# eridgd/WCT-TF

Measured on AMD Instinct MI355X. Metric: stylized frames/sec @512x512, 5-level relu5->1 pipeline, alpha=0.8, higher is better.
Workload: dtype f16

## Files before the change

### wct_tf_amd/csrc/api.hip

```cpp
#include "common.h"
#include "../../include/wct_hip.h"

#include <stdarg.h>
#include <stdio.h>
#include <string.h>
#include <stdlib.h>
#include <vector>
#include <cmath>
#include <algorithm>

static thread_local char g_err[512] = "";
void wct_set_error(const char* fmt, ...) {
  va_list ap;
  va_start(ap, fmt);
  vsnprintf(g_err, sizeof(g_err), fmt, ap);
  va_end(ap);
}
extern "C" const char* wct_last_error(void) { return g_err; }

struct DevBuf {
  void* p = nullptr;
  size_t cap = 0;
};

// ... 458 lines not shown
  ProfScope ps(c, conv3x3_wino_takes(a) ? 9 : 0, 2.0 * px * 9 * l.cin * l.cout,
               in_px * l.cin * 2 + out_px * l.cout * ((y16 ? 2 : 0) + (y32 ? 4 : 0)) + 9.0 * l.cin * l.cout * 2);
  return launch_conv3x3(a, c->stream);
}

static int run_encoder(wct_ctx* c, const float* img, int B, int H, int W, int clamp01, int deepest,
                       float* const taps32[6], float* const* usum = nullptr, unsigned* const* umax = nullptr) {
  if (!c->enc_loaded) { wct_set_error("encoder weights not set (wct_set_encoder)"); return WCT_ERR_STATE; }
  ARG_CHECK(deepest >= 1 && deepest <= 5 && H >= 2 && W >= 2);
  const size_t act_bytes = (size_t)B * H * W * 64 * sizeof(half_t);
  TRY(ensure(c, c->act[0], act_bytes));
  TRY(ensure(c, c->act[1], act_bytes));
  half_t* cur = (half_t*)c->act[0].p;
  half_t* nxt = (half_t*)c->act[1].p;
  static const int fuse_conv1_env = getenv("WCT_FUSE_CONV1") ? atoi(getenv("WCT_FUSE_CONV1")) : 1;
  const bool fuse_conv1 = fuse_conv1_env && deepest > 1 && !taps32[1];
  if (!fuse_conv1) {
    ConvFirstArgs a;
    a.x = img; a.wfrag = c->first_w; a.bias = c->first_b;
    a.y16 = deepest > 1 ? cur : nullptr; a.y32 = taps32[1];
    a.B = B; a.H = H; a.W = W; a.clamp01 = clamp01;
    a.usum = usum && taps32[1] ? usum[1] : nullptr; a.umax = a.usum ? umax[1] : nullptr;
    const double px = (double)B * H * W;
    ProfScope ps(c, 1, 2.0 * px * 27 * 64, px * (12 + 64 * ((a.y16 ? 2 : 0) + (a.y32 ? 4 : 0))));
    TRY(launch_conv_first(a, c->stream));
  }
  if (deepest == 1) return WCT_OK;
  static const int seq_tap[12] = {0, 2, 0, 3, 0, 0, 0, 4, 0, 0, 0, 5};
  static const int pool_after[12] = {1, 0, 1, 0, 0, 0, 1, 0, 0, 0, 1, 0};
  int h = H, w = W;
  for (int i = 0; i < 12; ++i) {
    const ConvLayer& l = c->enc[i];
    const int tap = seq_tap[i];
    const bool last = tap == deepest;
    const bool fuse = pool_after[i];
    float* const us = tap && taps32[tap] && usum ? usum[tap] : nullptr;
    if (i == 0 && fuse_conv1) {
      ConvArgs a;
      a.x = nullptr; a.w = l.w; a.bias = l.b; a.y16 = nxt; a.y32 = nullptr; a.usum = nullptr; a.umax = nullptr;
// ... 54 lines not shown
  const int mode = (flags & WCT_FLAG_MODE_NP) ? WCT_MODE_NP : WCT_MODE_TF;
  {
    ProfScope ps(c, 4, cost.cov_flops, cost.cov_bytes);
    TRY(launch(mode, WCT_STAGE_COV));
  }
  {
    ProfScope ps(c, 5, 0, 0);
    TRY(launch(mode, WCT_STAGE_EIG));
  }
  ProfScope ps(c, 6, cost.apply_flops, cost.apply_bytes);
  return launch(mode, WCT_STAGE_APPLY);
}

static int run_transform(wct_ctx* c, const float* fc, int Nc, const float* fs, int Ns, int C, int P,
                         float alpha, unsigned flags, float eps, half_t* out16, float* out32, int* sweeps_dev,
                         const WctFeatStats* st = nullptr) {
  const int shared = (flags & WCT_FLAG_STYLE_SHARED) ? 1 : 0;
  const StageCost cost = {(double)P * 2.0 * C * C * ((double)Nc + Ns), (double)P * 2.0 * ((double)Nc + Ns) * C * 4,
                          (double)P * (2.0 * C * C * Nc + 6.0 * C * C * C), (double)P * Nc * C * (4 + (out16 ? 2 : 0) + (out32 ? 4 : 0)),
                          (double)P * (2.0 * Nc + 2.0 * Ns) * C * 4 + (double)P * Nc * C * 6};
  return run_stages(c, wct_workspace_bytes(C, Nc, Ns, P), flags, cost, [&](int mode, int stages) {
    if (!stages) return launch_adain(fc, Nc, fs, Ns, C, P, alpha, 1e-5f, out16, out32, c->wct_ws.p, c->wct_ws.cap, c->stream, shared, st);
    return launch_wct(fc, Nc, fs, Ns, C, P, alpha, mode, eps, out16, out32, c->wct_ws.p, c->wct_ws.cap, sweeps_dev, stages, c->stream,
                      shared, c->eig_fail_dev, st);
  });
}

static int mix_weights(const float* weights, int K, float* lambda) {
  if (K < 1 || K > WCT_MIX_MAX) { wct_set_error("style mix: K = %d styles, must be 1 .. %d", K, (int)WCT_MIX_MAX); return WCT_ERR_ARG; }
  if (!weights) { wct_set_error("style mix: no weights"); return WCT_ERR_ARG; }
  double sum = 0.0;
  for (int k = 0; k < K; ++k) {
    if (!(weights[k] >= 0.f) || !std::isfinite(weights[k])) {
      wct_set_error("style mix: weight %d is %g; weights must be finite and >= 0", k, (double)weights[k]);
      return WCT_ERR_ARG;
    }
    sum += weights[k];
  }
  if (!(sum > 0.0) || !std::isfinite(sum)) { wct_set_error("style mix: the weights sum to %g, must be > 0", sum); return WCT_ERR_ARG; }
// ... 460 lines not shown
  if (flags & WCT_FLAG_IMAGES_F32) return WCT_OK;
  TRY(ensure(c, c->img_c, nc * 4));
  TRY(ensure(c, c->img_s, ns * 4));
  ProfScope ps(c, 7, 0, (double)(nc + ns) * 5);
  TRY(launch_u8_to_f32((const uint8_t*)content, (float*)c->img_c.p, nc, c->stream));
  TRY(launch_u8_to_f32((const uint8_t*)style, (float*)c->img_s.p, ns, c->stream));
  *img_c = (const float*)c->img_c.p; *img_s = (const float*)c->img_s.p;
  return WCT_OK;
}

static bool fuse_stats() {
  static const int on = getenv("WCT_FUSE_STATS") ? atoi(getenv("WCT_FUSE_STATS")) : 1;
  return on != 0;
}

template <typename StyleAt, typename Transform>
static int stylize_levels(wct_ctx* c, const float* img_c, int B, int Hc, int Wc, const int* levels, int n_levels, unsigned flags,
                          size_t umax_clear, int clear_from, StyleAt&& style_at, Transform&& transform, uint8_t* out) {
  unsigned* const umax_c = (unsigned*)c->umax.p;
  const float* cur = img_c;
  int H = Hc, W = Wc;
  for (int i = 0; i < n_levels; ++i) {
    const int l = levels[i], C = LEVEL_C[l];
    int h, w;
    level_dims(H, W, l, &h, &w);
    TRY(ensure(c, c->feat_c, (size_t)B * h * w * C * 4));
    float* ctaps[6] = {nullptr, nullptr, nullptr, nullptr, nullptr, nullptr};
    ctaps[l] = (float*)c->feat_c.p;
    float* us_c[6] = {nullptr, nullptr, nullptr, nullptr, nullptr, nullptr};
    unsigned* um_c[6] = {nullptr, nullptr, nullptr, nullptr, nullptr, nullptr};
    if (fuse_stats() && w % 16 == 0) {
      TRY(ensure(c, c->usum_c, (size_t)B * h * (w / 16) * C * 4));
      us_c[l] = (float*)c->usum_c.p; um_c[l] = umax_c;
      if (i >= clear_from) HIP_TRY(hipMemsetAsync(umax_c, 0, umax_clear, c->stream));
    }
    WctFeatStats st = {};
    st.u[0] = us_c[l]; st.umax[0] = um_c[l];
    TRY(run_encoder(c, cur, B, H, W, i > 0, l, ctaps, us_c, um_c));
    TRY(ensure(c, c->wct_out, (size_t)B * h * w * C * 2));
    if (l == 5 && (flags & WCT_FLAG_SWAP5)) {
      int hs, ws;
      style_at(l, 0, &hs, &ws);
      ARG_CHECK(h >= c->ss_patch && w >= c->ss_patch && hs >= c->ss_patch && ws >= c->ss_patch);
// ... 24 lines not shown
  int deepest, Ho, Wo;
  TRY(stylize_checks(c, Hc, Wc, &style, &Hs, &Ws, 1, levels, n_levels, &deepest, &Ho, &Wo));

  const int shared = (flags & WCT_FLAG_STYLE_SHARED) ? 1 : 0;
  const int Bs = shared ? 1 : B;
  const float *img_c, *img_s;
  TRY(images_f32(c, flags, content, (size_t)B * Hc * Wc * 3, style, (size_t)Bs * Hs * Ws * 3, &img_c, &img_s));
  const bool want_stats = fuse_stats();
  constexpr size_t UROW = 32 * UMAX_SLOTS;
  TRY(ensure(c, c->umax, 7 * UROW * sizeof(unsigned)));
  unsigned* const umax_c = (unsigned*)c->umax.p;
  if (want_stats) HIP_TRY(hipMemsetAsync(c->umax.p, 0, 7 * UROW * sizeof(unsigned), c->stream));
  float* taps[6] = {nullptr, nullptr, nullptr, nullptr, nullptr, nullptr};
  float* us_s[6] = {nullptr, nullptr, nullptr, nullptr, nullptr, nullptr};
  unsigned* um_s[6] = {nullptr, nullptr, nullptr, nullptr, nullptr, nullptr};
  for (int i = 0; i < n_levels; ++i) {
    const int l = levels[i];
    int h, w;
    level_dims(Hs, Ws, l, &h, &w);
    TRY(ensure(c, c->feat_s[l], (size_t)Bs * h * w * LEVEL_C[l] * 4));
    taps[l] = (float*)c->feat_s[l].p;
    if (want_stats && w % 16 == 0) {
      TRY(ensure(c, c->usum_s[l], (size_t)Bs * h * (w / 16) * LEVEL_C[l] * 4));
      us_s[l] = (float*)c->usum_s[l].p; um_s[l] = umax_c + UROW * l;
    }
  }
  TRY(run_encoder(c, img_s, Bs, Hs, Ws, 0, deepest, taps, us_s, um_s));

  auto style_at = [&](int l, int b, int* hs, int* ws) {
    level_dims(Hs, Ws, l, hs, ws);
    return (const float*)c->feat_s[l].p + (size_t)(shared ? 0 : b) * *hs * *ws * LEVEL_C[l];
  };
  return stylize_levels(c, img_c, B, Hc, Wc, levels, n_levels, flags, UROW * sizeof(unsigned), 1, style_at,
                        [&](int, int l, int C, int h, int w, WctFeatStats st) {
                          int hs, ws;
                          const float* fs = style_at(l, 0, &hs, &ws);
                          st.u[1] = us_s[l]; st.umax[1] = um_s[l];
                          return run_transform(c, (float*)c->feat_c.p, h * w, fs, hs * ws, C, B, alpha, flags, -1.f,
                                               (half_t*)c->wct_out.p, nullptr, nullptr, &st);
                        }, out);
}

extern "C" int wct_stylize(wct_ctx* c, const uint8_t* content, int Hc, int Wc, const uint8_t* style, int Hs, int Ws,
                           const int* levels, int n_levels, float alpha, unsigned flags, uint8_t* out) {
  ARG_CHECK(c && content && style && out);
  HIP_TRY(hipSetDevice(c->device));
  TRY(eig_stale(c));
  int Ho, Wo;
  TRY(wct_output_size(Hc, Wc, levels, n_levels, &Ho, &Wo));
  void *dc, *ds;
  const size_t px = (flags & WCT_FLAG_IMAGES_F32) ? sizeof(float) : 1;
  TRY(stage_in(c, 0, content, (size_t)Hc * Wc * 3 * px, &dc));
  TRY(stage_in(c, 1, style, (size_t)Hs * Ws * 3 * px, &ds));
  TRY(ensure(c, c->stage[2], (size_t)Ho * Wo * 3));
  TRY(wct_stylize_batch_dev(c, (uint8_t*)dc, Hc, Wc, (uint8_t*)ds, Hs, Ws, 1, levels, n_levels, alpha, flags,
// ... 383 lines not shown
```

### wct_tf_amd/csrc/common.h

```cpp
#pragma once
#include <hip/hip_runtime.h>
#include <stdint.h>
#include <stddef.h>

typedef _Float16 half_t;
typedef _Float16 half8 __attribute__((ext_vector_type(8)));
typedef _Float16 half4 __attribute__((ext_vector_type(4)));
typedef float f32x16 __attribute__((ext_vector_type(16)));
typedef float f32x4 __attribute__((ext_vector_type(4)));

#define WCT_OK 0
#define WCT_ERR_HIP -1
#define WCT_ERR_ARG -2
#define WCT_ERR_STATE -3
#define WCT_ERR_NOMEM -4
#define WCT_ERR_NOCONV -5

void wct_set_error(const char* fmt, ...);

#define HIP_TRY(expr)                                                          \
  do {                                                                         \
    hipError_t _e = (expr);                                                    \
    if (_e != hipSuccess) {                                                    \
      wct_set_error("%s failed: %s (%s:%d)", #expr, hipGetErrorString(_e),     \
// ... 106 lines not shown
  int nsplit;
  size_t sA, sB, s_sub_m, s_sub_n, s_sub_k, s_scale_k, s_out, s_bias;
  const float* A_odd;
  size_t sA_odd;
  int skip_shared;
  int blend; float alpha; unsigned* mabs;
  const float* mask_diag; size_t s_mask; int* mask_out; const int* mask_in;
};

int launch_gemm(GemmArgs g, int nsplit, int nbatch, hipStream_t s);

enum { WCT_MODE_NP = 0, WCT_MODE_TF = 1 };

struct WctFeatStats { const float* u[2]; const unsigned* umax[2]; };

size_t wct_workspace_bytes(int C, int Nc, int Ns, int P);
int launch_wct(const float* content, int Nc, const float* style, int Ns, int C, int P,
               float alpha, int mode, float eps , half_t* out16, float* out32,
               void* workspace, size_t workspace_bytes, int* sweeps_dev, int stages, hipStream_t s,
               int shared_style ,
               int* eig_fail ,
               const struct WctFeatStats* stats = nullptr );
enum { WCT_STAGE_COV = 1, WCT_STAGE_EIG = 2, WCT_STAGE_APPLY = 4, WCT_STAGE_ALL = 7, WCT_STAGE_EIG_FP32UPDATE = 8 };
int launch_adain(const float* content, int Nc, const float* style, int Ns, int C, int P,
                 float alpha, float eps, half_t* out16, float* out32,
                 void* workspace, size_t workspace_bytes, hipStream_t s, int shared_style,
                 const struct WctFeatStats* stats = nullptr);
enum { WCT_MIX_MAX = 8 };
size_t wct_mix_workspace_bytes(int C, int Nc, const int* Ns, int K, const float* lambda);
int launch_wct_mix(const float* content, int Nc, const float* const* styles, const int* Ns, int K, const float* lambda, int C,
                   float alpha, int mode, float eps, half_t* out16, float* out32, void* workspace, size_t workspace_bytes,
                   int* sweeps_dev, int stages, hipStream_t s, int* eig_fail, const struct WctFeatStats* stats = nullptr);
int launch_adain_mix(const float* content, int Nc, const float* const* styles, const int* Ns, int K, const float* lambda, int C,
                     float alpha, float eps, half_t* out16, float* out32, void* workspace, size_t workspace_bytes, hipStream_t s,
                     const struct WctFeatStats* stats = nullptr);
struct MaskGeom { const uint8_t* mask; int Hm, Wm, w, stride; };
size_t mask_compact_workspace_bytes(int N);
// ... 50 lines not shown
```

### wct_tf_amd/csrc/conv.hip

```cpp
#include "common.h"

typedef unsigned int u32x4 __attribute__((ext_vector_type(4)));
constexpr int TW = 16;
constexpr int PITCH = 20;
constexpr int BK = 32;

__device__ __forceinline__ int reflect_idx(int i, int n) {
  if (i < 0) i = -i;
  if (i >= n) i = 2 * n - 2 - i;
  i = i < 0 ? 0 : i;
  return i >= n ? n - 1 : i;
}

template <int MT, int NT, bool POOL, bool OUT32>
__device__ __forceinline__ void conv_epilogue_t(const ConvArgs& p, f32x16 (&acc)[NT][MT], int b, int y0, int x0, int n0,
                                                int wm, int wn, int lane, const unsigned char* bias_lds) {
  typedef _Float16 h2 __attribute__((ext_vector_type(2)));
  constexpr int OOB = (int)0x80000000u;
  const int frag_px = lane & 15;
  const int frag_py = (lane & 31) >> 4;
  const int kgrp = lane >> 5;
  const int Ho = POOL ? (p.H + 1) / 2 : p.H, Wo = POOL ? (p.W + 1) / 2 : p.W;
  const unsigned img_elems = (unsigned)Ho * Wo * p.Cout;
  const __amdgpu_buffer_rsrc_t r16 = __builtin_amdgcn_make_buffer_rsrc(
// ... 581 lines not shown
    }
    __builtin_amdgcn_fence(__ATOMIC_RELEASE, "wavefront");
    __builtin_amdgcn_wave_barrier();
  }
  if (next) {
    __syncthreads();
    park();
    __syncthreads();
  }
  }
  if (p.usum) umax_merge(p.umax + b * UMAX_SLOTS, (int)blockIdx.x * 4 + wave, vmax, lane);
}

int launch_conv_first(const ConvFirstArgs& a, hipStream_t s) {
  ARG_CHECK(a.H > 1 && a.W > 1 && a.B > 0);
  ARG_CHECK(!a.usum || (a.y32 && a.umax && a.W % 16 == 0));
  const int strips_x = cdiv(a.W, 64), tiles_y = cdiv(a.H, 16);
  hipLaunchKernelGGL(conv_first_kernel, dim3(strips_x * tiles_y, a.B), dim3(256), 0, s, a, strips_x);
  HIP_TRY(hipGetLastError());
  return WCT_OK;
}

__global__ __launch_bounds__(256) void conv_last_kernel(ConvLastArgs p, int tiles_x) {
  constexpr int PP = 33;
  __shared__ float part[18 * 18 * PP];
  const int tid = threadIdx.x, lane = tid & 63, wave = tid >> 6;
  const int tx = blockIdx.x % tiles_x, ty = blockIdx.x / tiles_x;
  const int b = blockIdx.y;
  const int y0 = ty * 16, x0 = tx * 16;
  const half_t* xb = p.x + (size_t)b * p.H * p.W * 64;
  half8 wf[4];
// ... 130 lines not shown
```

### wct_tf_amd/csrc/stats_gemm.hip

```cpp
#include "wct_stages.h"


struct StatArgs {
  const float* x[2];
  int n[2];
  const float* u[2];
  const unsigned* umax[2];
  const float* mean;
  float* partial;
  float* absmax;
  int C, nslab;
  int shared_style;
};

__global__ __launch_bounds__(256) void colsum_kernel(StatArgs p) {
  __shared__ f32x4 red[256];
  const int mat = blockIdx.y, slab = blockIdx.x;
  if (skip_style_mat(mat, p.shared_style)) return;
  const int b = mat & 1, pair = mat >> 1;
  const int C = p.C, cq = C / 4;
  const int nrp = 256 / cq;
  const int tid = threadIdx.x;
  const int rp = tid / cq, c4 = tid % cq;
  const int N = p.n[b];
// ... 489 lines not shown
    CovArgs ca;
    ca.x[0] = content; ca.x[1] = style; ca.n[0] = Nc; ca.n[1] = Ns;
    ca.mean = w.mean; ca.scale = w.scale; ca.partial = w.cov_partial;
    ca.C = C; ca.ksplit = w.ksplit; ca.nsplit = w.nsplit; ca.ntile = cdiv(C, BT); ca.shared_style = shared_style;
    dim3 grid(ca.ntile * (ca.ntile + 1) / 2, w.nsplit, 2 * P);
    if (BT == 128) hipLaunchKernelGGL((cov_f16x2_kernel<128>), grid, dim3(256), 0, s, ca);
    else hipLaunchKernelGGL((cov_f16x2_kernel<64>), grid, dim3(256), 0, s, ca);
    HIP_TRY(hipGetLastError());
  }
  hipLaunchKernelGGL(cov_finish_kernel, dim3(cdiv(C, 64), cdiv(C, 64), 2 * P), dim3(256), 0, s, w.cov_partial, w.scale, w.A, C,
                     w.nsplit, BT, 1.f / (float)(Nc - 1), 1.f / (float)(Ns - 1), eps, shared_style, w.A0);
  HIP_TRY(hipGetLastError());
  return WCT_OK;
}

static int launch_slot_means(const float* x, int N, int C, int m, int nslab, const WctCarve& w, bool with_var, hipStream_t s,
                             const float* u = nullptr, const unsigned* umax = nullptr) {
  StatArgs sa = {};
  sa.x[0] = sa.x[1] = x; sa.n[0] = sa.n[1] = N;
  sa.u[0] = umax ? u : nullptr; sa.umax[0] = sa.u[0] ? umax : nullptr;
  float* partial = w.stat_partial + (size_t)m * w.nslab * C;
  float* absmax = w.absmax + (size_t)m * w.nslab;
  sa.mean = nullptr; sa.partial = partial; sa.absmax = absmax; sa.C = C; sa.nslab = nslab; sa.shared_style = 0;
  hipLaunchKernelGGL(colsum_kernel, dim3(nslab, 1), dim3(256), 0, s, sa);
  hipLaunchKernelGGL(colsum_finish_kernel, dim3(cdiv(C, 256), 1), dim3(256), 0, s, partial, w.mean + (size_t)m * C, C, nslab, (float)N,
                     (float)N, 0, (const float*)absmax, w.scale + m);
  if (with_var) {
    sa.mean = w.mean + (size_t)m * C; sa.absmax = nullptr;
    hipLaunchKernelGGL(colsum_kernel, dim3(nslab, 1), dim3(256), 0, s, sa);
    hipLaunchKernelGGL(colsum_finish_kernel, dim3(cdiv(C, 256), 1), dim3(256), 0, s, partial, w.var + (size_t)m * C, C, nslab, (float)N,
// ... 33 lines not shown
```

### wct_tf_amd/csrc/wct.hip

```cpp
#include "wct_stages.h"
#include "jacobi_dev.h"
#include <algorithm>
#include <type_traits>



template <int BC, int BP, typename Args = ApplyArgs>
__global__ __launch_bounds__(256, 2) void apply_f16x2_kernel(Args p) {
  constexpr bool SEG = std::is_same<Args, ApplySegArgs>::value;
  constexpr int TM = BC / 64, TN = BP / 64;
  constexpr int MI = BC * 4 / 256, XI = BP * 4 / 256;
  __shared__ __attribute__((aligned(16))) unsigned char lm[2][BC * 64];
  __shared__ __attribute__((aligned(16))) unsigned char lx[2][BP * 64];
  typedef unsigned int u32x4 __attribute__((ext_vector_type(4)));
  const int tid = threadIdx.x, lane = tid & 63, wave = tid >> 6;
  const int wm = wave >> 1, wn = wave & 1;
  const int pair = blockIdx.z;
  const int n0 = blockIdx.x * BP, c0 = blockIdx.y * BC;
  int seg0 = 0, N = p.N;
  if constexpr (SEG) {
    seg0 = p.seg_off[p.lab[pair]];
    N = p.seg_off[p.lab[pair] + 1] - seg0;
    if (n0 >= N) return;
  }
// ... 134 lines not shown
        typedef _Float16 h2 __attribute__((ext_vector_type(2)));
        h2 lo = {(half_t)v[0], (half_t)v[1]}, hi = {(half_t)v[2], (half_t)v[3]};
        pk[rq][0] = __builtin_bit_cast(unsigned, lo);
        pk[rq][1] = __builtin_bit_cast(unsigned, hi);
      }
      if (p.out16) {
#pragma unroll
        for (int m = 0; m < 2; ++m) {
          auto sxw = __builtin_amdgcn_permlane32_swap(pk[2 * m][0], pk[2 * m + 1][0], false, false);
          auto syw = __builtin_amdgcn_permlane32_swap(pk[2 * m][1], pk[2 * m + 1][1], false, false);
          u32x4 o = {sxw[0], syw[0], sxw[1], syw[1]};
          const int co = cb + 16 * m + 8 * kgrp;
          if (n_ok && co < C) *reinterpret_cast<u32x4*>(p.out16 + row + co) = o;
        }
      }
    }
  }
}

int launch_apply_seg(const ApplySegArgs& a, int nmax, int P, hipStream_t s) {
  const int C = a.C;
  if (C >= 128) hipLaunchKernelGGL((apply_f16x2_kernel<128, 128, ApplySegArgs>), dim3(cdiv(nmax, 128), cdiv(C, 128), P), dim3(256), 0, s, a);
  else hipLaunchKernelGGL((apply_f16x2_kernel<64, 128, ApplySegArgs>), dim3(cdiv(nmax, 128), cdiv(C, 64), P), dim3(256), 0, s, a);
  HIP_TRY(hipGetLastError());
  return WCT_OK;
}

static int wct_nslab(int N) { int s = cdiv(N, 64); return s < 1 ? 1 : (s > 256 ? 256 : s); }

static void cov_split(int C, int Nmax, int P, int* nsplit, int* ksplit) {
// ... 52 lines not shown
size_t wct_workspace_bytes(int C, int Nc, int Ns, int P) {
  const int Cw = C < 32 ? 32 : C;
  return carve(nullptr, Cw, P, pair_layout(Cw, Nc, Ns)).total;
}

int launch_blend(const WctCarve& w, int C, int P, float alpha, int shared_style, hipStream_t s) {
  const size_t cc = (size_t)C * C;
  GemmArgs g = {};
  g.A = w.Tcs; g.lda = C; g.a_kmajor = 0; g.B = w.Tw; g.ldb = C; g.b_kmajor = 1; g.sA = shared_style ? 0 : 2 * cc; g.sB = 2 * cc;
  g.M = C; g.N = C; g.K = C; g.ksplit = C; g.out32 = w.M; g.ldo = C; g.s_out = cc;
  g.blend = 1; g.alpha = alpha; g.mabs = w.mabs;
  return launch_gemm(g, 1, P, s);
}

static int launch_blend_apply(const WctCarve& w, const float* content, int Nc, int C, int P, float alpha, int shared_style,
                              half_t* out16, float* out32, hipStream_t s) {
  int rc;
  if ((rc = launch_blend(w, C, P, alpha, shared_style, s))) return rc;
  {
    ApplyArgs a;
    a.x = content; a.N = Nc; a.C = C; a.mean = w.mean; a.M = w.M; a.bias = w.bias;
    a.xscale = w.scale; a.mabs = w.mabs; a.out16 = out16; a.out32 = out32;
    if (C >= 128) hipLaunchKernelGGL((apply_f16x2_kernel<128, 128>), dim3(cdiv(Nc, 128), cdiv(C, 128), P), dim3(256), 0, s, a);
    else hipLaunchKernelGGL((apply_f16x2_kernel<64, 128>), dim3(cdiv(Nc, 128), cdiv(C, 64), P), dim3(256), 0, s, a);
  }
  HIP_TRY(hipGetLastError());
  return WCT_OK;
}

int launch_wct(const float* content, int Nc, const float* style, int Ns, int C, int P, float alpha, int mode, float eps_in,
               half_t* out16, float* out32, void* workspace, size_t workspace_bytes, int* sweeps_dev,
               int stages, hipStream_t s, int shared_style, int* eig_fail, const WctFeatStats* stats) {
  ARG_CHECK(C % 32 == 0 && C >= 32 && C <= 1024 && Nc >= 2 && Ns >= 2 && P >= 1 && P <= 32);
  ARG_CHECK(mode == WCT_MODE_NP || mode == WCT_MODE_TF);
  ARG_CHECK((size_t)Nc * C * 4 < ((size_t)1 << 31) && (size_t)Ns * C * 4 < ((size_t)1 << 31));
  WctCarve w = carve(workspace, C, P, pair_layout(C, Nc, Ns));
  ARG_CHECK(workspace_bytes >= w.total);
  int rc;
  if (stages & WCT_STAGE_COV) {
    if ((rc = launch_means(content, Nc, style, Ns, C, P, w, false, shared_style, s, stats))) return rc;
    if ((rc = launch_cov(content, Nc, style, Ns, C, P, w, cov_eps(mode, eps_in), shared_style, s))) return rc;
  }
  if ((stages & WCT_STAGE_EIG) &&
      (rc = launch_eig_stage(w, C, P, shared_style, (stages & WCT_STAGE_EIG_FP32UPDATE) ? 0 : 1, sweeps_dev, eig_fail, s)))
    return rc;
  if (!(stages & WCT_STAGE_APPLY)) return WCT_OK;

  if ((rc = launch_spectral_tail(w, C, P, alpha, mode, eps_in, shared_style, P, s))) return rc;
  return launch_blend_apply(w, content, Nc, C, P, alpha, shared_style, out16, out32, s);
}

void plan_carve(SlotPlan* sp, void* base, int C) {
  PairLayout mx = {1, 1, 0};
  for (int m = 0; m < 2 * sp->P; ++m)
    if (sp->slot[m].n) { mx.nslab = std::max(mx.nslab, sp->slot[m].lay.nslab); mx.nsplit = std::max(mx.nsplit, sp->slot[m].lay.nsplit); }
  sp->w = carve(base, C, std::max(sp->P, 1), mx);
  sp->total = sp->w.total;
}

bool plan_fits(const SlotPlan& sp, int C) {
  for (int m = 0; m < 2 * sp.P; ++m)
    if ((size_t)sp.slot[m].n * C * 4 >= ((size_t)1 << 31)) return false;
  return true;
}
// ... 147 lines not shown
```

### wct_tf_amd/csrc/wct_stages.h

```cpp
#pragma once
#include "common.h"

constexpr int WCT_SKIP_MIX = 2;
__device__ __host__ __forceinline__ bool skip_style_mat(int mat, int shared_style) {
  return shared_style == WCT_SKIP_MIX ? ((mat & 1) == 0 && mat > 0) : (shared_style && (mat & 1) && mat > 1);
}

constexpr int EIG_CORRECT = 2;
constexpr float JACOBI_TOL_FN = 1.5e-2f;
constexpr float JACOBI_TOL_FN2 = 4e-2f;
constexpr float JACOBI_TOL_FN_WCT = EIG_CORRECT >= 2 ? JACOBI_TOL_FN2 : (EIG_CORRECT ? JACOBI_TOL_FN : 0.f);

static inline size_t align_up(size_t x) { return (x + 255) & ~(size_t)255; }

struct WctCarve {
  float *mean, *var, *stat_partial, *absmax, *scale, *cov_partial, *A, *A0, *V, *d, *G, *X, *S2, *Tw, *Tcs, *T, *M, *bias, *mix;
  unsigned* mabs; int* refresh;
  void* jacobi_ws; size_t jacobi_bytes;
  int nslab, nsplit, ksplit;
  size_t total;
};

struct PairLayout { int nslab, nsplit, ksplit; };
PairLayout pair_layout(int C, int Nc, int Ns);
// ... 16 lines not shown
  size_t total;
};
void plan_carve(SlotPlan* sp, void* base, int C);
bool plan_fits(const SlotPlan& sp, int C);

struct ApplyArgs {
  const float* x; int N; int C;
  const float* mean;
  const float* M; const float* bias;
  const float* xscale;
  const unsigned* mabs;
  half_t* out16; float* out32;
};
struct ApplySegArgs : ApplyArgs { const int* seg_off; const int* perm; int lab[WCT_MIX_MAX]; };

int launch_means(const float* content, int Nc, const float* style, int Ns, int C, int P, const WctCarve& w, bool with_var,
                 int shared_style, hipStream_t s, const WctFeatStats* fs = nullptr);
int launch_cov(const float* content, int Nc, const float* style, int Ns, int C, int P, const WctCarve& w, float eps, int shared_style,
               hipStream_t s);
int launch_plan_stats(const SlotPlan& sp, int C, bool with_var, bool with_cov, float eps, hipStream_t s);
int launch_eig_stage(const WctCarve& w, int C, int P, int skip, int u_f16, int* sweeps_dev, int* eig_fail, hipStream_t s);
int launch_refresh(const WctCarve& w, int C, int P, int shared_style, hipStream_t s, bool always = false);
int launch_spectral_tail(const WctCarve& w, int C, int P, float alpha, int mode, float eps_in, int shared_style, int nwhite, hipStream_t s);
int launch_spectral_function(const float* A, const float* V, float* G, float* X, float* out, int C, int nbatch, size_t stride,
                             size_t out_stride, int kind, float shift, hipStream_t s, float* scratch2 = nullptr);
int launch_blend(const WctCarve& w, int C, int P, float alpha, int shared_style, hipStream_t s);
int launch_apply_seg(const ApplySegArgs& a, int nmax, int P, hipStream_t s);
```

Measured before the change: 672.9.

## Recompute level-1 conv features inside WCT covariance and apply kernels

For the relu1 level, the full-resolution 64-channel fp32 feature maps are no longer written out for content and style. The covariance and apply kernels instead gather the RGB image, recompute the first 3x3 conv on the fly with split-f16 MFMA, and feed the result straight into the covariance GEMM or the whitening/coloring GEMM. Means still come from the row-sum stats that conv_first now emits without an fp32 tap. This cuts large feature-map writes and reads at 512x512. The cost is repeating the first-layer conv twice, once for covariance and once for apply, and adding new kernels with only a narrow set of supported shapes.

```diff
diff --git a/wct_tf_amd/csrc/api.hip b/wct_tf_amd/csrc/api.hip
--- a/wct_tf_amd/csrc/api.hip
+++ b/wct_tf_amd/csrc/api.hip
@@ -496,15 +496,16 @@
   half_t* cur = (half_t*)c->act[0].p;
   half_t* nxt = (half_t*)c->act[1].p;
   static const int fuse_conv1_env = getenv("WCT_FUSE_CONV1") ? atoi(getenv("WCT_FUSE_CONV1")) : 1;
-  const bool fuse_conv1 = fuse_conv1_env && deepest > 1 && !taps32[1];
+  float* const usum1 = usum ? usum[1] : nullptr;
+  const bool fuse_conv1 = fuse_conv1_env && deepest > 1 && !taps32[1] && !usum1;
   if (!fuse_conv1) {
     ConvFirstArgs a;
     a.x = img; a.wfrag = c->first_w; a.bias = c->first_b;
     a.y16 = deepest > 1 ? cur : nullptr; a.y32 = taps32[1];
     a.B = B; a.H = H; a.W = W; a.clamp01 = clamp01;
-    a.usum = usum && taps32[1] ? usum[1] : nullptr; a.umax = a.usum ? umax[1] : nullptr;
+    a.usum = usum1; a.umax = a.usum ? umax[1] : nullptr;
     const double px = (double)B * H * W;
-    ProfScope ps(c, 1, 2.0 * px * 27 * 64, px * (12 + 64 * ((a.y16 ? 2 : 0) + (a.y32 ? 4 : 0))));
+    ProfScope ps(c, 1, 2.0 * px * 27 * 64, px * (12 + 64 * ((a.y16 ? 2 : 0) + (a.y32 ? 4 : 0)) + (a.usum ? 16 : 0)));
     TRY(launch_conv_first(a, c->stream));
   }
   if (deepest == 1) return WCT_OK;
@@ -589,15 +590,17 @@
 
 static int run_transform(wct_ctx* c, const float* fc, int Nc, const float* fs, int Ns, int C, int P,
                          float alpha, unsigned flags, float eps, half_t* out16, float* out32, int* sweeps_dev,
-                         const WctFeatStats* st = nullptr) {
+                         const WctFeatStats* st = nullptr, const WctLevel1Src* level1 = nullptr) {
   const int shared = (flags & WCT_FLAG_STYLE_SHARED) ? 1 : 0;
-  const StageCost cost = {(double)P * 2.0 * C * C * ((double)Nc + Ns), (double)P * 2.0 * ((double)Nc + Ns) * C * 4,
-                          (double)P * (2.0 * C * C * Nc + 6.0 * C * C * C), (double)P * Nc * C * (4 + (out16 ? 2 : 0) + (out32 ? 4 : 0)),
+  const double in_px = level1 ? 12.0 : C * 4.0, l1_flops = level1 ? 2.0 * 27 * 64 : 0.0;
+  const StageCost cost = {(double)P * (2.0 * C * C + l1_flops) * ((double)Nc + Ns), (double)P * ((double)Nc + Ns) * (level1 ? 12.0 + C * 4.0 / 16 : 2.0 * C * 4),
+                          (double)P * ((2.0 * C * C + l1_flops) * Nc + 6.0 * C * C * C),
+                          (double)P * Nc * (in_px + C * ((out16 ? 2 : 0) + (out32 ? 4 : 0))),
                           (double)P * (2.0 * Nc + 2.0 * Ns) * C * 4 + (double)P * Nc * C * 6};
   return run_stages(c, wct_workspace_bytes(C, Nc, Ns, P), flags, cost, [&](int mode, int stages) {
     if (!stages) return launch_adain(fc, Nc, fs, Ns, C, P, alpha, 1e-5f, out16, out32, c->wct_ws.p, c->wct_ws.cap, c->stream, shared, st);
     return launch_wct(fc, Nc, fs, Ns, C, P, alpha, mode, eps, out16, out32, c->wct_ws.p, c->wct_ws.cap, sweeps_dev, stages, c->stream,
-                      shared, c->eig_fail_dev, st);
+                      shared, c->eig_fail_dev, st, level1);
   });
 }
 
@@ -1088,9 +1091,27 @@
   return on != 0;
 }
 
+static bool level1_from_images(unsigned flags, int Hc, int Wc, int Ws, const int* levels, int n_levels) {
+  static const int on = getenv("WCT_FUSE_LEVEL1") ? atoi(getenv("WCT_FUSE_LEVEL1")) : 1;
+  if (!on || !fuse_stats() || (flags & WCT_FLAG_ADAIN)) return false;
+  bool any = false;
+  int H = Hc, W = Wc;
+  for (int i = 0; i < n_levels; ++i) {
+    int h, w;
+    level_dims(H, W, levels[i], &h, &w);
+    if (levels[i] == 1) {
+      if (!wct_level1_takes(w, Ws)) return false;
+      any = true;
+    }
+    H = h << (levels[i] - 1); W = w << (levels[i] - 1);
+  }
+  return any;
+}
+
 template <typename StyleAt, typename Transform>
 static int stylize_levels(wct_ctx* c, const float* img_c, int B, int Hc, int Wc, const int* levels, int n_levels, unsigned flags,
-                          size_t umax_clear, int clear_from, StyleAt&& style_at, Transform&& transform, uint8_t* out) {
+                          size_t umax_clear, int clear_from, StyleAt&& style_at, Transform&& transform, uint8_t* out,
+                          WctLevel1Src* level1 = nullptr) {
   unsigned* const umax_c = (unsigned*)c->umax.p;
   const float* cur = img_c;
   int H = Hc, W = Wc;
@@ -1098,9 +1119,14 @@
     const int l = levels[i], C = LEVEL_C[l];
     int h, w;
     level_dims(H, W, l, &h, &w);
-    TRY(ensure(c, c->feat_c, (size_t)B * h * w * C * 4));
+    const bool from_image = level1 && l == 1;
     float* ctaps[6] = {nullptr, nullptr, nullptr, nullptr, nullptr, nullptr};
-    ctaps[l] = (float*)c->feat_c.p;
+    if (from_image) {
+      level1->img[0] = cur; level1->H[0] = H; level1->W[0] = W; level1->clamp01 = i > 0;
+    } else {
+      TRY(ensure(c, c->feat_c, (size_t)B * h * w * C * 4));
+      ctaps[l] = (float*)c->feat_c.p;
+    }
     float* us_c[6] = {nullptr, nullptr, nullptr, nullptr, nullptr, nullptr};
     unsigned* um_c[6] = {nullptr, nullptr, nullptr, nullptr, nullptr, nullptr};
     if (fuse_stats() && w % 16 == 0) {
@@ -1155,12 +1181,20 @@
   float* taps[6] = {nullptr, nullptr, nullptr, nullptr, nullptr, nullptr};
   float* us_s[6] = {nullptr, nullptr, nullptr, nullptr, nullptr, nullptr};
   unsigned* um_s[6] = {nullptr, nullptr, nullptr, nullptr, nullptr, nullptr};
+  WctLevel1Src level1 = {};
+  const bool from_images = level1_from_images(flags, Hc, Wc, Ws, levels, n_levels);
+  if (from_images) {
+    level1.img[1] = img_s; level1.H[1] = Hs; level1.W[1] = Ws;
+    level1.wfrag = c->first_w; level1.bias = c->first_b;
+  }
   for (int i = 0; i < n_levels; ++i) {
     const int l = levels[i];
     int h, w;
     level_dims(Hs, Ws, l, &h, &w);
-    TRY(ensure(c, c->feat_s[l], (size_t)Bs * h * w * LEVEL_C[l] * 4));
-    taps[l] = (float*)c->feat_s[l].p;
+    if (!(from_images && l == 1)) {
+      TRY(ensure(c, c->feat_s[l], (size_t)Bs * h * w * LEVEL_C[l] * 4));
+      taps[l] = (float*)c->feat_s[l].p;
+    }
     if (want_stats && w % 16 == 0) {
       TRY(ensure(c, c->usum_s[l], (size_t)Bs * h * (w / 16) * LEVEL_C[l] * 4));
       us_s[l] = (float*)c->usum_s[l].p; um_s[l] = umax_c + UROW * l;
@@ -1177,9 +1211,12 @@
                           int hs, ws;
                           const float* fs = style_at(l, 0, &hs, &ws);
                           st.u[1] = us_s[l]; st.umax[1] = um_s[l];
+                          if (from_images && l == 1)
+                            return run_transform(c, nullptr, h * w, nullptr, hs * ws, C, B, alpha, flags, -1.f,
+                                                 (half_t*)c->wct_out.p, nullptr, nullptr, &st, &level1);
                           return run_transform(c, (float*)c->feat_c.p, h * w, fs, hs * ws, C, B, alpha, flags, -1.f,
                                                (half_t*)c->wct_out.p, nullptr, nullptr, &st);
-                        }, out);
+                        }, out, from_images ? &level1 : nullptr);
 }
 
 extern "C" int wct_stylize(wct_ctx* c, const uint8_t* content, int Hc, int Wc, const uint8_t* style, int Hs, int Ws,
diff --git a/wct_tf_amd/csrc/common.h b/wct_tf_amd/csrc/common.h
--- a/wct_tf_amd/csrc/common.h
+++ b/wct_tf_amd/csrc/common.h
@@ -144,13 +144,17 @@
 
 struct WctFeatStats { const float* u[2]; const unsigned* umax[2]; };
 
+struct WctLevel1Src { const float* img[2]; int H[2], W[2]; int clamp01; const half_t* wfrag; const float* bias; };
+static inline bool wct_level1_takes(int Wc, int Ws) { return Wc % 32 == 0 && Ws % 32 == 0; }
+
 size_t wct_workspace_bytes(int C, int Nc, int Ns, int P);
 int launch_wct(const float* content, int Nc, const float* style, int Ns, int C, int P,
                float alpha, int mode, float eps , half_t* out16, float* out32,
                void* workspace, size_t workspace_bytes, int* sweeps_dev, int stages, hipStream_t s,
                int shared_style ,
                int* eig_fail ,
-               const struct WctFeatStats* stats = nullptr );
+               const struct WctFeatStats* stats = nullptr ,
+               const struct WctLevel1Src* level1 = nullptr );
 enum { WCT_STAGE_COV = 1, WCT_STAGE_EIG = 2, WCT_STAGE_APPLY = 4, WCT_STAGE_ALL = 7, WCT_STAGE_EIG_FP32UPDATE = 8 };
 int launch_adain(const float* content, int Nc, const float* style, int Ns, int C, int P,
                  float alpha, float eps, half_t* out16, float* out32,
diff --git a/wct_tf_amd/csrc/conv.hip b/wct_tf_amd/csrc/conv.hip
--- a/wct_tf_amd/csrc/conv.hip
+++ b/wct_tf_amd/csrc/conv.hip
@@ -619,7 +619,7 @@
 
 int launch_conv_first(const ConvFirstArgs& a, hipStream_t s) {
   ARG_CHECK(a.H > 1 && a.W > 1 && a.B > 0);
-  ARG_CHECK(!a.usum || (a.y32 && a.umax && a.W % 16 == 0));
+  ARG_CHECK(!a.usum || (a.umax && a.W % 16 == 0));
   const int strips_x = cdiv(a.W, 64), tiles_y = cdiv(a.H, 16);
   hipLaunchKernelGGL(conv_first_kernel, dim3(strips_x * tiles_y, a.B), dim3(256), 0, s, a, strips_x);
   HIP_TRY(hipGetLastError());
diff --git a/wct_tf_amd/csrc/stats_gemm.hip b/wct_tf_amd/csrc/stats_gemm.hip
--- a/wct_tf_amd/csrc/stats_gemm.hip
+++ b/wct_tf_amd/csrc/stats_gemm.hip
@@ -527,6 +527,127 @@
   return WCT_OK;
 }
 
+struct CovL1Args {
+  WctLevel1Src src;
+  const float* mean;
+  const float* scale;
+  float* partial;
+  int ksplit, nsplit, shared_style;
+};
+
+__global__ __launch_bounds__(256, 2) void cov_level1_kernel(CovL1Args p) {
+  constexpr int C = 64, NS = 4;
+  __shared__ __attribute__((aligned(16))) unsigned char lds[NS][2][C * 64];
+  typedef unsigned u32x2 __attribute__((ext_vector_type(2)));
+  typedef _Float16 h2 __attribute__((ext_vector_type(2)));
+  const int tid = threadIdx.x, lane = tid & 63, wave = __builtin_amdgcn_readfirstlane(tid >> 6);
+  const int wm = wave >> 1, wn = wave & 1;
+  const int mat = blockIdx.z, split = blockIdx.y;
+  if (skip_style_mat(mat, p.shared_style)) return;
+  const int side = mat & 1, pair = mat >> 1;
+  const int H = p.src.H[side], W = p.src.W[side], N = H * W;
+  const float* img = p.src.img[side] + (size_t)pair * N * 3;
+  const int clamp01 = side == 0 ? p.src.clamp01 : 0;
+  const int kbeg = split * p.ksplit;
+  const int kend = min(N, kbeg + p.ksplit);
+  const float sc = p.scale[mat];
+  const int l31 = lane & 31, kgrp = lane >> 5;
+
+  L1Weights wts;
+  l1_load_weights(p.src.wfrag, lane, wts);
+  float bias[2], mean[2];
+#pragma unroll
+  for (int nt = 0; nt < 2; ++nt) {
+    bias[nt] = p.src.bias[nt * 32 + l31];
+    mean[nt] = p.mean[mat * C + nt * 32 + l31];
+  }
+  f32x16 acc;
+#pragma unroll
+  for (int r = 0; r < 16; ++r) acc[r] = 0.f;
+
+  float raw[2][8];
+  auto gather = [&](int k0) {
+    const int s0 = k0 + wave * 32;
+    if (s0 < kend) {
+      const int y = s0 / W;
+      l1_gather(img, H, W, y, s0 - y * W + l31, kgrp, raw);
+    }
+  };
+  if (kbeg < kend) gather(kbeg);
+  for (int k0 = kbeg; k0 < kend; k0 += 32 * NS) {
+    if (k0 + wave * 32 < kend) {
+      half8 bh[2], bl[2];
+      l1_split(raw, clamp01, bh, bl);
+      if (k0 + 32 * NS < kend) gather(k0 + 32 * NS);
+#pragma unroll
+      for (int nt = 0; nt < 2; ++nt) {
+        const f32x16 a = l1_conv<true>(wts, nt, bh, bl);
+        const int c = nt * 32 + l31;
+#pragma unroll
+        for (int rq = 0; rq < 4; ++rq) {
+          half_t h[4], l[4];
+#pragma unroll
+          for (int j = 0; j < 4; ++j) {
+            const float x = fmaxf(a[rq * 4 + j] + bias[nt], 0.f);
+            const float v = (x - mean[nt]) * sc;
+            h[j] = (half_t)v;
+            l[j] = (half_t)(v - (float)h[j]);
+          }
+          const int off = (c * 4 + (rq ^ ((c >> 2) & 3))) * 16 + kgrp * 8;
+          *reinterpret_cast<u32x2*>(lds[wave][0] + off) =
+              u32x2{__builtin_bit_cast(unsigned, h2{h[0], h[1]}), __builtin_bit_cast(unsigned, h2{h[2], h[3]})};
+          *reinterpret_cast<u32x2*>(lds[wave][1] + off) =
+              u32x2{__builtin_bit_cast(unsigned, h2{l[0], l[1]}), __builtin_bit_cast(unsigned, h2{l[2], l[3]})};
+        }
+      }
+    }
+    __syncthreads();
+    const int nst = min(NS, (kend - k0) >> 5);
+#pragma unroll
+    for (int st = 0; st < NS; ++st) {
+      if (st >= nst) break;
+#pragma unroll
+      for (int ks = 0; ks < 2; ++ks) {
+        const int chunk = ks * 2 + kgrp;
+        const int ra = wm * 32 + l31, rb = wn * 32 + l31;
+        const int offa = (ra * 4 + (chunk ^ ((ra >> 2) & 3))) * 16, offb = (rb * 4 + (chunk ^ ((rb >> 2) & 3))) * 16;
+        const half8 ah = *reinterpret_cast<const half8*>(lds[st][0] + offa);
+        const half8 al = *reinterpret_cast<const half8*>(lds[st][1] + offa);
+        const half8 bhf = *reinterpret_cast<const half8*>(lds[st][0] + offb);
+        const half8 blf = *reinterpret_cast<const half8*>(lds[st][1] + offb);
+        acc = __builtin_amdgcn_mfma_f32_32x32x16_f16(al, bhf, acc, 0, 0, 0);
+        acc = __builtin_amdgcn_mfma_f32_32x32x16_f16(ah, blf, acc, 0, 0, 0);
+        acc = __builtin_amdgcn_mfma_f32_32x32x16_f16(ah, bhf, acc, 0, 0, 0);
+      }
+    }
+    __syncthreads();
+  }
+
+  float* out = p.partial + ((size_t)mat * p.nsplit + split) * C * C;
+  const int gn = wn * 32 + l31;
+#pragma unroll
+  for (int r = 0; r < 16; ++r) {
+    const int gm = wm * 32 + (r & 3) + 8 * (r >> 2) + 4 * kgrp;
+    out[(size_t)gm * C + gn] = acc[r];
+  }
+}
+
+int launch_cov_level1(const WctLevel1Src& src, int P, const WctCarve& w, float eps, int shared_style, hipStream_t s) {
+  constexpr int C = 64;
+  const int Nc = src.H[0] * src.W[0], Ns = src.H[1] * src.W[1];
+  ARG_CHECK(src.img[0] && src.img[1] && src.wfrag && src.bias && wct_level1_takes(src.W[0], src.W[1]) && src.H[0] >= 2 && src.H[1] >= 2);
+  ARG_CHECK(w.ksplit % 32 == 0);
+  CovL1Args ca;
+  ca.src = src; ca.mean = w.mean; ca.scale = w.scale; ca.partial = w.cov_partial;
+  ca.ksplit = w.ksplit; ca.nsplit = w.nsplit; ca.shared_style = shared_style;
+  hipLaunchKernelGGL(cov_level1_kernel, dim3(1, w.nsplit, 2 * P), dim3(256), 0, s, ca);
+  HIP_TRY(hipGetLastError());
+  hipLaunchKernelGGL(cov_finish_kernel, dim3(1, 1, 2 * P), dim3(256), 0, s, w.cov_partial, w.scale, w.A, C,
+                     w.nsplit, 64, 1.f / (float)(Nc - 1), 1.f / (float)(Ns - 1), eps, shared_style, w.A0);
+  HIP_TRY(hipGetLastError());
+  return WCT_OK;
+}
+
 static int launch_slot_means(const float* x, int N, int C, int m, int nslab, const WctCarve& w, bool with_var, hipStream_t s,
                              const float* u = nullptr, const unsigned* umax = nullptr) {
   StatArgs sa = {};
diff --git a/wct_tf_amd/csrc/wct.hip b/wct_tf_amd/csrc/wct.hip
--- a/wct_tf_amd/csrc/wct.hip
+++ b/wct_tf_amd/csrc/wct.hip
@@ -172,6 +172,160 @@
           if (n_ok && co < C) *reinterpret_cast<u32x4*>(p.out16 + row + co) = o;
         }
       }
+    }
+  }
+}
+
+struct ApplyL1Args {
+  WctLevel1Src src;
+  const float* mean; const float* M; const float* bias; const float* xscale; const unsigned* mabs;
+  half_t* out16;
+};
+
+__global__ __launch_bounds__(256, 2) void apply_level1_kernel(ApplyL1Args p) {
+  constexpr int C = 64, BP = 128, TN = 2;
+  __shared__ __attribute__((aligned(16))) unsigned char lm[2][2][C * 64];
+  __shared__ __attribute__((aligned(16))) unsigned char lx[2][2][BP * 64];
+  typedef unsigned int u32x4 __attribute__((ext_vector_type(4)));
+  typedef unsigned u32x2 __attribute__((ext_vector_type(2)));
+  typedef _Float16 h2 __attribute__((ext_vector_type(2)));
+  const int tid = threadIdx.x, lane = tid & 63, wave = __builtin_amdgcn_readfirstlane(tid >> 6);
+  const int wm = wave >> 1, wn = wave & 1;
+  const int pair = blockIdx.z;
+  const int n0 = blockIdx.x * BP;
+  const int H = p.src.H[0], W = p.src.W[0], N = H * W;
+  const float* img = p.src.img[0] + (size_t)pair * N * 3;
+  const float* M = p.M + (size_t)pair * C * C;
+  const float* mean = p.mean + (size_t)pair * 2 * C;
+  const float sx = p.xscale[2 * pair];
+  float sM = 1.f;
+  {
+    const float m = __uint_as_float(p.mabs[pair]);
+    if (m > 0.f) { int e; frexpf(m, &e); sM = ldexpf(1.f, 14 - e); }
+  }
+  const int l31 = lane & 31, kgrp = lane >> 5;
+
+  float raw[2][8];
+  const int s0 = n0 + wave * 32;
+  if (s0 < N) {
+    const int y = s0 / W;
+    l1_gather(img, H, W, y, s0 - y * W + l31, kgrp, raw);
+  }
+  {
+    const int row = tid >> 2, kq = tid & 3;
+    const int moff = (row * 4 + (kq ^ ((row >> 2) & 3))) * 16;
+#pragma unroll
+    for (int kst = 0; kst < 2; ++kst) {
+      const f32x4 r0 = *reinterpret_cast<const f32x4*>(M + row * C + kq * 8 + kst * 32);
+      const f32x4 r1 = *reinterpret_cast<const f32x4*>(M + row * C + kq * 8 + kst * 32 + 4);
+      half8 h, l;
+#pragma unroll
+      for (int j = 0; j < 8; ++j) {
+        const float v = (j < 4 ? r0[j & 3] : r1[j & 3]) * sM;
+        h[j] = (half_t)v;
+        l[j] = (half_t)(v - (float)h[j]);
+      }
+      *reinterpret_cast<half8*>(lm[kst][0] + moff) = h;
+      *reinterpret_cast<half8*>(lm[kst][1] + moff) = l;
+    }
+  }
+  if (s0 < N) {
+    L1Weights wts;
+    l1_load_weights(p.src.wfrag, lane, wts);
+    half8 bh[2], bl[2];
+    l1_split(raw, p.src.clamp01, bh, bl);
+    const int row = wave * 32 + l31;
+#pragma unroll
+    for (int nt = 0; nt < 2; ++nt) {
+      const f32x16 a = l1_conv<false>(wts, nt, bh, bl);
+#pragma unroll
+      for (int rq = 0; rq < 4; ++rq) {
+        const int ch = nt * 32 + 8 * rq + 4 * kgrp;
+        const f32x4 b4 = *reinterpret_cast<const f32x4*>(p.src.bias + ch);
+        const f32x4 m4 = *reinterpret_cast<const f32x4*>(mean + ch);
+        f32x4 x;
+#pragma unroll
+        for (int j = 0; j < 4; ++j) x[j] = fmaxf(a[rq * 4 + j] + b4[j], 0.f);
+        const f32x4 rx = x - m4;
+        half_t h[4], l[4];
+#pragma unroll
+        for (int j = 0; j < 4; ++j) {
+          const float v = rx[j] * sx;
+          h[j] = (half_t)v;
+          l[j] = (half_t)(v - (float)h[j]);
+        }
+        const int off = (row * 4 + (rq ^ ((row >> 2) & 3))) * 16 + kgrp * 8;
+        *reinterpret_cast<u32x2*>(lx[nt][0] + off) =
+            u32x2{__builtin_bit_cast(unsigned, h2{h[0], h[1]}), __builtin_bit_cast(unsigned, h2{h[2], h[3]})};
+        *reinterpret_cast<u32x2*>(lx[nt][1] + off) =
+            u32x2{__builtin_bit_cast(unsigned, h2{l[0], l[1]}), __builtin_bit_cast(unsigned, h2{l[2], l[3]})};
+      }
+    }
+  }
+  __syncthreads();
+
+  f32x16 acc[TN];
+#pragma unroll
+  for (int j = 0; j < TN; ++j)
+#pragma unroll
+    for (int r = 0; r < 16; ++r) acc[j][r] = 0.f;
+#pragma unroll
+  for (int kst = 0; kst < 2; ++kst)
+#pragma unroll
+    for (int ks = 0; ks < 2; ++ks) {
+      const int chunk = ks * 2 + kgrp;
+      const int r = wm * 32 + l31;
+      const int off = (r * 4 + (chunk ^ ((r >> 2) & 3))) * 16;
+      const half8 ah = *reinterpret_cast<const half8*>(lm[kst][0] + off);
+      const half8 al = *reinterpret_cast<const half8*>(lm[kst][1] + off);
+      half8 xh[TN], xl[TN];
+#pragma unroll
+      for (int j = 0; j < TN; ++j) {
+        const int rp = (wn * TN + j) * 32 + l31;
+        const int offx = (rp * 4 + (chunk ^ ((rp >> 2) & 3))) * 16;
+        xh[j] = *reinterpret_cast<const half8*>(lx[kst][0] + offx);
+        xl[j] = *reinterpret_cast<const half8*>(lx[kst][1] + offx);
+      }
+#pragma unroll
+      for (int j = 0; j < TN; ++j) {
+        acc[j] = __builtin_amdgcn_mfma_f32_32x32x16_f16(al, xh[j], acc[j], 0, 0, 0);
+        acc[j] = __builtin_amdgcn_mfma_f32_32x32x16_f16(ah, xl[j], acc[j], 0, 0, 0);
+        acc[j] = __builtin_amdgcn_mfma_f32_32x32x16_f16(ah, xh[j], acc[j], 0, 0, 0);
+      }
+    }
+
+  const float inv = 1.f / (sx * sM);
+  const float* bias = p.bias + (size_t)pair * C;
+  f32x4 bvs[4];
+#pragma unroll
+  for (int rq = 0; rq < 4; ++rq) bvs[rq] = *reinterpret_cast<const f32x4*>(bias + wm * 32 + 8 * rq + 4 * kgrp);
+#pragma unroll
+  for (int j = 0; j < TN; ++j) {
+    const int n = n0 + (wn * TN + j) * 32 + l31;
+    const bool n_ok = n < N;
+    const size_t row = ((size_t)pair * N + (n_ok ? n : 0)) * C;
+    const int cb = wm * 32;
+    unsigned pk[4][2];
+#pragma unroll
+    for (int rq = 0; rq < 4; ++rq) {
+      const f32x4 bv = bvs[rq];
+      f32x4 v;
+#pragma unroll
+      for (int q = 0; q < 4; ++q) {
+        v[q] = acc[j][rq * 4 + q] * inv + bv[q];
+        asm volatile("" : "+v"(v[q]));
+      }
+      h2 lo = {(half_t)v[0], (half_t)v[1]}, hi = {(half_t)v[2], (half_t)v[3]};
+      pk[rq][0] = __builtin_bit_cast(unsigned, lo);
+      pk[rq][1] = __builtin_bit_cast(unsigned, hi);
+    }
+#pragma unroll
+    for (int m = 0; m < 2; ++m) {
+      auto sxw = __builtin_amdgcn_permlane32_swap(pk[2 * m][0], pk[2 * m + 1][0], false, false);
+      auto syw = __builtin_amdgcn_permlane32_swap(pk[2 * m][1], pk[2 * m + 1][1], false, false);
+      u32x4 o = {sxw[0], syw[0], sxw[1], syw[1]};
+      const int co = cb + 16 * m + 8 * kgrp;
+      if (n_ok) *reinterpret_cast<u32x4*>(p.out16 + row + co) = o;
     }
   }
 }
@@ -254,10 +408,14 @@
 }
 
 static int launch_blend_apply(const WctCarve& w, const float* content, int Nc, int C, int P, float alpha, int shared_style,
-                              half_t* out16, float* out32, hipStream_t s) {
+                              half_t* out16, float* out32, hipStream_t s, const WctLevel1Src* level1 = nullptr) {
   int rc;
   if ((rc = launch_blend(w, C, P, alpha, shared_style, s))) return rc;
-  {
+  if (level1) {
+    ApplyL1Args a;
+    a.src = *level1; a.mean = w.mean; a.M = w.M; a.bias = w.bias; a.xscale = w.scale; a.mabs = w.mabs; a.out16 = out16;
+    hipLaunchKernelGGL(apply_level1_kernel, dim3(cdiv(Nc, 128), 1, P), dim3(256), 0, s, a);
+  } else {
     ApplyArgs a;
     a.x = content; a.N = Nc; a.C = C; a.mean = w.mean; a.M = w.M; a.bias = w.bias;
     a.xscale = w.scale; a.mabs = w.mabs; a.out16 = out16; a.out32 = out32;
@@ -270,8 +428,10 @@
 
 int launch_wct(const float* content, int Nc, const float* style, int Ns, int C, int P, float alpha, int mode, float eps_in,
                half_t* out16, float* out32, void* workspace, size_t workspace_bytes, int* sweeps_dev,
-               int stages, hipStream_t s, int shared_style, int* eig_fail, const WctFeatStats* stats) {
+               int stages, hipStream_t s, int shared_style, int* eig_fail, const WctFeatStats* stats, const WctLevel1Src* level1) {
   ARG_CHECK(C % 32 == 0 && C >= 32 && C <= 1024 && Nc >= 2 && Ns >= 2 && P >= 1 && P <= 32);
+  ARG_CHECK(!level1 || (C == 64 && Nc == level1->H[0] * level1->W[0] && Ns == level1->H[1] * level1->W[1] && !out32 && out16 &&
+                        stats && stats->u[0] && stats->umax[0] && stats->u[1] && stats->umax[1]));
   ARG_CHECK(mode == WCT_MODE_NP || mode == WCT_MODE_TF);
   ARG_CHECK((size_t)Nc * C * 4 < ((size_t)1 << 31) && (size_t)Ns * C * 4 < ((size_t)1 << 31));
   WctCarve w = carve(workspace, C, P, pair_layout(C, Nc, Ns));
@@ -279,7 +439,9 @@
   int rc;
   if (stages & WCT_STAGE_COV) {
     if ((rc = launch_means(content, Nc, style, Ns, C, P, w, false, shared_style, s, stats))) return rc;
-    if ((rc = launch_cov(content, Nc, style, Ns, C, P, w, cov_eps(mode, eps_in), shared_style, s))) return rc;
+    if ((rc = level1 ? launch_cov_level1(*level1, P, w, cov_eps(mode, eps_in), shared_style, s)
+                     : launch_cov(content, Nc, style, Ns, C, P, w, cov_eps(mode, eps_in), shared_style, s)))
+      return rc;
   }
   if ((stages & WCT_STAGE_EIG) &&
       (rc = launch_eig_stage(w, C, P, shared_style, (stages & WCT_STAGE_EIG_FP32UPDATE) ? 0 : 1, sweeps_dev, eig_fail, s)))
@@ -287,7 +449,7 @@
   if (!(stages & WCT_STAGE_APPLY)) return WCT_OK;
 
   if ((rc = launch_spectral_tail(w, C, P, alpha, mode, eps_in, shared_style, P, s))) return rc;
-  return launch_blend_apply(w, content, Nc, C, P, alpha, shared_style, out16, out32, s);
+  return launch_blend_apply(w, content, Nc, C, P, alpha, shared_style, out16, out32, s, level1);
 }
 
 void plan_carve(SlotPlan* sp, void* base, int C) {
diff --git a/wct_tf_amd/csrc/wct_stages.h b/wct_tf_amd/csrc/wct_stages.h
--- a/wct_tf_amd/csrc/wct_stages.h
+++ b/wct_tf_amd/csrc/wct_stages.h
@@ -54,10 +54,77 @@
 };
 struct ApplySegArgs : ApplyArgs { const int* seg_off; const int* perm; int lab[WCT_MIX_MAX]; };
 
+__device__ __forceinline__ int l1_reflect(int i, int n) {
+  i = i < 0 ? -i : i;
+  return i >= n ? 2 * n - 2 - i : i;
+}
+__device__ __forceinline__ void l1_gather(const float* img, int H, int W, int y, int x, int kgrp, float (&raw)[2][8]) {
+  int row[3], col[3];
+#pragma unroll
+  for (int d = 0; d < 3; ++d) {
+    row[d] = l1_reflect(y - 1 + d, H) * W * 3;
+    col[d] = l1_reflect(x - 1 + d, W) * 3;
+  }
+#pragma unroll
+  for (int ks = 0; ks < 2; ++ks)
+#pragma unroll
+    for (int j = 0; j < 8; ++j) {
+      const int k0 = 16 * ks + j, k1 = k0 + 8;
+      const int off0 = row[k0 / 9] + col[(k0 % 9) / 3] + k0 % 3;
+      if (k1 < 27) {
+        const int off1 = row[k1 / 9] + col[(k1 % 9) / 3] + k1 % 3;
+        raw[ks][j] = img[kgrp ? off1 : off0];
+      } else {
+        const float v = img[off0];
+        raw[ks][j] = kgrp ? 0.f : v;
+      }
+    }
+}
+__device__ __forceinline__ void l1_split(const float (&raw)[2][8], int clamp01, half8 (&bh)[2], half8 (&bl)[2]) {
+#pragma unroll
+  for (int ks = 0; ks < 2; ++ks)
+#pragma unroll
+    for (int j = 0; j < 8; ++j) {
+      const float v = clamp01 ? fminf(fmaxf(raw[ks][j], 0.f), 1.f) : raw[ks][j];
+      bh[ks][j] = (half_t)v;
+      bl[ks][j] = (half_t)(v - (float)bh[ks][j]);
+    }
+}
+struct L1Weights { half8 wh[2][2], wl[2][2]; };
+__device__ __forceinline__ void l1_load_weights(const half_t* wfrag, int lane, L1Weights& w) {
+#pragma unroll
+  for (int t = 0; t < 2; ++t)
+#pragma unroll
+    for (int ks = 0; ks < 2; ++ks) {
+      w.wh[t][ks] = *reinterpret_cast<const half8*>(wfrag + (((t * 2 + ks) * 2 + 0) * 64 + lane) * 8);
+      w.wl[t][ks] = *reinterpret_cast<const half8*>(wfrag + (((t * 2 + ks) * 2 + 1) * 64 + lane) * 8);
+    }
+}
+template <bool TRANSPOSED>
+__device__ __forceinline__ f32x16 l1_conv(const L1Weights& w, int nt, const half8 (&bh)[2], const half8 (&bl)[2]) {
+  f32x16 a;
+#pragma unroll
+  for (int r = 0; r < 16; ++r) a[r] = 0.f;
+#pragma unroll
+  for (int ks = 0; ks < 2; ++ks) {
+    if (TRANSPOSED) {
+      a = __builtin_amdgcn_mfma_f32_32x32x16_f16(bh[ks], w.wl[nt][ks], a, 0, 0, 0);
+      a = __builtin_amdgcn_mfma_f32_32x32x16_f16(bl[ks], w.wh[nt][ks], a, 0, 0, 0);
+      a = __builtin_amdgcn_mfma_f32_32x32x16_f16(bh[ks], w.wh[nt][ks], a, 0, 0, 0);
+    } else {
+      a = __builtin_amdgcn_mfma_f32_32x32x16_f16(w.wl[nt][ks], bh[ks], a, 0, 0, 0);
+      a = __builtin_amdgcn_mfma_f32_32x32x16_f16(w.wh[nt][ks], bl[ks], a, 0, 0, 0);
+      a = __builtin_amdgcn_mfma_f32_32x32x16_f16(w.wh[nt][ks], bh[ks], a, 0, 0, 0);
+    }
+  }
+  return a;
+}
+
 int launch_means(const float* content, int Nc, const float* style, int Ns, int C, int P, const WctCarve& w, bool with_var,
                  int shared_style, hipStream_t s, const WctFeatStats* fs = nullptr);
 int launch_cov(const float* content, int Nc, const float* style, int Ns, int C, int P, const WctCarve& w, float eps, int shared_style,
                hipStream_t s);
+int launch_cov_level1(const WctLevel1Src& src, int P, const WctCarve& w, float eps, int shared_style, hipStream_t s);
 int launch_plan_stats(const SlotPlan& sp, int C, bool with_var, bool with_cov, float eps, hipStream_t s);
 int launch_eig_stage(const WctCarve& w, int C, int P, int skip, int u_f16, int* sweeps_dev, int* eig_fail, hipStream_t s);
 int launch_refresh(const WctCarve& w, int C, int P, int shared_style, hipStream_t s, bool always = false);
```

Result: no change. 676.3, median of 6 (+0.5%).
